# ZhangHaoyang493/News_Recsys

Measured on AMD Instinct MI355X. Metric: impressions/sec at batch 65536 (embedding hot path forward), higher is better.
Workload: dtype f32

## Files before the change

news_recsys_amd/csrc/nrx_interact.hip:

```cpp
#include "nrx_common.h"

namespace {

__global__ __launch_bounds__(NRX_BLOCK) void bag_pool_fwd_kernel(const float* __restrict__ emb, const float* __restrict__ mask,
                                                                 int64_t batch, int L, int D, float* __restrict__ out) {
    const int64_t total = batch * (int64_t)D;
    for (int64_t i = (int64_t)blockIdx.x * NRX_BLOCK + threadIdx.x; i < total; i += (int64_t)gridDim.x * NRX_BLOCK) {
        const int64_t b = i / D;
        const int d = (int)(i - b * D);
        const float* e = emb + (b * L) * (int64_t)D + d;
        float acc = 0.f, den = 0.f;
        if (mask != nullptr) {
            const float* m = mask + b * (int64_t)L;
            for (int l = 0; l < L; ++l) {
#pragma clang fp contract(off)
                const float w = m[l];
                den += w;
                acc += e[(int64_t)l * D] * w;
            }
            out[i] = acc / (den + 1e-8f);
        } else {
            for (int l = 0; l < L; ++l) acc += e[(int64_t)l * D];
            out[i] = acc / (float)L;
        }
    }
}

template <bool VEC>
__global__ __launch_bounds__(NRX_BLOCK) void bag_pool_bwd_kernel(const float* __restrict__ g_out, const float* __restrict__ mask,
                                                                 int64_t batch, int L, int D, float* __restrict__ g_emb) {
    const int lane = threadIdx.x & 63;
    const int64_t wave = (int64_t)blockIdx.x * (NRX_BLOCK / 64) + (threadIdx.x >> 6);
    const int64_t nwaves = (int64_t)gridDim.x * (NRX_BLOCK / 64);
    const int n = L * D;
    for (int64_t b = wave; b < batch; b += nwaves) {
        float den = (float)L;
        if (mask != nullptr) {
            float part = 0.f;
            for (int l = lane; l < L; l += NRX_WAVE) part += mask[b * (int64_t)L + l];
            den = nrx_wave_sum(part) + 1e-8f;
        }
        const float* gb = g_out + b * (int64_t)D;
        const float* mb = mask ? mask + b * (int64_t)L : nullptr;
        float* ob = g_emb + b * (int64_t)n;
        if (VEC) {
            const unsigned q = (unsigned)D >> 2;
            for (unsigned e4 = lane; e4 < (unsigned)n >> 2; e4 += NRX_WAVE) {
                const unsigned l = e4 / q, d = (e4 - l * q) * 4;
                const float4 g = *reinterpret_cast<const float4*>(gb + d);
                const float m = mb ? mb[l] : 1.0f;
                float4 o = make_float4(g.x / den, g.y / den, g.z / den, g.w / den);
                if (mb) o = make_float4(o.x * m, o.y * m, o.z * m, o.w * m);
                *reinterpret_cast<float4*>(ob + (size_t)e4 * 4) = o;
            }
        } else {
            for (int e = lane; e < n; e += NRX_WAVE) {
                const int l = e / D, d = e - l * D;
                const float g = gb[d] / den;
                ob[e] = mb ? g * mb[l] : g;
            }
        }
    }
}

__device__ __forceinline__ float4 ld4(const float* p, int k0, int D, bool vec) {
    float4 v;
    if (vec) {
        v = *reinterpret_cast<const float4*>(p);
    } else {
        v.x = p[0];
        v.y = (k0 + 1 < D) ? p[1] : 0.f;
        v.z = (k0 + 2 < D) ? p[2] : 0.f;
        v.w = (k0 + 3 < D) ? p[3] : 0.f;
    }
    return v;
}

template <int QLOG2>
__global__ __launch_bounds__(NRX_BLOCK) void fm_fwd_kernel(const float* __restrict__ feat, int64_t ld, int F, int D,
                                                           int64_t batch, float* __restrict__ fm_out, bool vec,
                                                           float* __restrict__ sums = nullptr, int64_t sums_ld = 0) {
    constexpr int Q = 1 << QLOG2;
    constexpr int TB = NRX_BLOCK / Q;
    const int q = threadIdx.x & (Q - 1);
    const int64_t b = (int64_t)blockIdx.x * TB + (threadIdx.x >> QLOG2);
    const bool live = b < batch;
    float total = 0.f;
    for (int kc = 0; kc < D; kc += 4 * Q) {
        const int k0 = kc + q * 4;
        float first = 0.f;
        float4 s = make_float4(0.f, 0.f, 0.f, 0.f), sq = s;
        if (live && k0 < D) {
            const float* row = feat + b * ld + k0;
            for (int f = 0; f < F; ++f) {
                float4 v = ld4(row + (int64_t)f * D, k0, D, vec);
                if (k0 == 0) { first += v.x; v.x = 0.f; }
                s.x += v.x; s.y += v.y; s.z += v.z; s.w += v.w;
                sq.x += v.x * v.x; sq.y += v.y * v.y; sq.z += v.z * v.z; sq.w += v.w * v.w;
            }
        }
        total += 0.5f * ((s.x * s.x - sq.x) + (s.y * s.y - sq.y) + (s.z * s.z - sq.z) + (s.w * s.w - sq.w)) + first;
        if (sums != nullptr && live && k0 < D) {
            float* dst = sums + b * sums_ld + k0;
            const float v0 = k0 == 0 ? first : s.x;
            dst[0] = v0;
            if (k0 + 1 < D) dst[1] = s.y;
            if (k0 + 2 < D) dst[2] = s.z;
            if (k0 + 3 < D) dst[3] = s.w;
        }
    }
#pragma unroll
    for (int off = Q / 2; off > 0; off >>= 1) total += __shfl_xor(total, off, 64);
    if (live && q == 0) fm_out[b] = total;
}

template <int QLOG2>
__global__ __launch_bounds__(NRX_BLOCK) void fm_bwd_kernel(const float* __restrict__ feat, int64_t ld, int F, int D, int64_t batch,
                                                           const float* __restrict__ g_fm, const float* g_in, int64_t g_in_ld,
                                                           float* g_feat, int64_t g_ld, bool vec) {
    constexpr int Q = 1 << QLOG2;
    constexpr int TB = NRX_BLOCK / Q;
    constexpr int U = 8;
    const int q = threadIdx.x & (Q - 1);
    const int64_t b = (int64_t)blockIdx.x * TB + (threadIdx.x >> QLOG2);
    if (b >= batch) return;
    const float gl = g_fm[b];
    const bool gvec = vec && (g_ld & 3) == 0 && ((reinterpret_cast<uintptr_t>(g_feat) & 15u) == 0) &&
                      (g_in == nullptr || ((g_in_ld & 3) == 0 && (reinterpret_cast<uintptr_t>(g_in) & 15u) == 0));
    for (int kc = 0; kc < D; kc += 4 * Q) {
        const int k0 = kc + q * 4;
        if (k0 >= D) continue;
        const float* row = feat + b * ld + k0;
        const float* irow = g_in ? g_in + b * g_in_ld + k0 : nullptr;
        float* grow = g_feat + b * g_ld + k0;
        float4 s = make_float4(0.f, 0.f, 0.f, 0.f);
        int f = 0;
        for (; f + U <= F; f += U) {
            float4 v[U];
#pragma unroll
            for (int u = 0; u < U; ++u) v[u] = ld4(row + (int64_t)(f + u) * D, k0, D, vec);
#pragma unroll
            for (int u = 0; u < U; ++u) { s.x += v[u].x; s.y += v[u].y; s.z += v[u].z; s.w += v[u].w; }
        }
        for (; f < F; ++f) {
            const float4 v = ld4(row + (int64_t)f * D, k0, D, vec);
            s.x += v.x; s.y += v.y; s.z += v.z; s.w += v.w;
        }
        f = 0;
        if (gvec && k0 + 4 <= D) {
            for (; f + U <= F; f += U) {
                float4 v[U], up[U];
#pragma unroll
                for (int u = 0; u < U; ++u) {
                    v[u] = ld4(row + (int64_t)(f + u) * D, k0, D, vec);
                    up[u] = irow ? *reinterpret_cast<const float4*>(irow + (int64_t)(f + u) * D) : make_float4(0.f, 0.f, 0.f, 0.f);
                }
#pragma unroll
                for (int u = 0; u < U; ++u) {
                    float4 g = make_float4(gl * (s.x - v[u].x), gl * (s.y - v[u].y), gl * (s.z - v[u].z), gl * (s.w - v[u].w));
                    if (k0 == 0) g.x = gl;
                    *reinterpret_cast<float4*>(grow + (int64_t)(f + u) * D) = make_float4(up[u].x + g.x, up[u].y + g.y, up[u].z + g.z, up[u].w + g.w);
                }
            }
        }
        for (; f < F; ++f) {
            const float4 v = ld4(row + (int64_t)f * D, k0, D, vec);
            float g[4] = {gl * (s.x - v.x), gl * (s.y - v.y), gl * (s.z - v.z), gl * (s.w - v.w)};
            if (k0 == 0) g[0] = gl;
            float* gp = grow + (int64_t)f * D;
            const float* ip = irow ? irow + (int64_t)f * D : nullptr;
#pragma unroll
            for (int j = 0; j < 4; ++j)
                if (k0 + j < D) gp[j] = (ip ? ip[j] : 0.f) + g[j];
        }
    }
}

template <int R, int V>
struct RowRegs {
    float v[R][V];
};

template <int R, int V>
__device__ __forceinline__ void row_load(RowRegs<R, V>& x, const float* p, int D, int lane) {
#pragma unroll
    for (int r = 0; r < R; ++r) {
        const int c = (r * 64 + lane) * V;
        if (V == 4) {
            float4 t = make_float4(0.f, 0.f, 0.f, 0.f);
            if (c < D) t = *reinterpret_cast<const float4*>(p + c);
            x.v[r][0] = t.x; x.v[r][1 % V] = t.y; x.v[r][2 % V] = t.z; x.v[r][3 % V] = t.w;
        } else {
            x.v[r][0] = (c < D) ? p[c] : 0.f;
        }
    }
}
// ... 499 lines not shown
                if (STNT) __builtin_nontemporal_store(t, o + u * Q + q);
                else o[u * Q + q] = t;
            }
        }
        float4 xl[N];
#pragma unroll
        for (int u = 0; u < N; ++u) xl[u] = x0[u];
        for (int l = 0; l < NL; ++l) {
            const float4* wl = s_w + l * (W / 4) + q;
            const float4* bl = s_b + l * (W / 4) + q;
            float part = 0.f;
#pragma unroll
            for (int u = 0; u < N; ++u) {
                const float4 wv = wl[u * Q];
                part += xl[u].x * wv.x + xl[u].y * wv.y + xl[u].z * wv.z + xl[u].w * wv.w;
            }
            const float dot = group_sum_dpp<Q>(part);
#pragma unroll
            for (int u = 0; u < N; ++u) {
                const float4 bv = bl[u * Q];
                xl[u].x = x0[u].x * dot + bv.x + xl[u].x;
                xl[u].y = x0[u].y * dot + bv.y + xl[u].y;
                xl[u].z = x0[u].z * dot + bv.z + xl[u].z;
                xl[u].w = x0[u].w * dot + bv.w + xl[u].w;
            }
        }
        if (live) {
            NRX_GLOBAL nrx_f32x4* o = (NRX_GLOBAL nrx_f32x4*)(a->out + b * a->out_ld);
#pragma unroll
            for (int u = EARLY ? N : 0; u < 2 * N; ++u) {
                const float4 v = u < N ? x0[u] : xl[u - N];
                nrx_f32x4 t;
                t.x = v.x; t.y = v.y; t.z = v.z; t.w = v.w;
                NRX_GLOBAL nrx_f32x4* dst = o + (u < N ? 0 : W / 4) + (u < N ? u : u - N) * Q + q;
                if (STNT) __builtin_nontemporal_store(t, dst);
                else *dst = t;
            }
        }
    }
}

int ceil_log2i(int x) {
    int l = 0;
    while ((1 << l) < x) ++l;
    return l;
}

unsigned stream_grid(int64_t items, int per_block) {
    int64_t g = (items + per_block - 1) / per_block;
    const int64_t cap = 256 * 8;
    if (g > cap) g = cap;
    if (g < 1) g = 1;
    return (unsigned)g;
}

#define NRX_QSWITCH(qlog2, ...)               \
    switch (qlog2) {                           \
        case 0: { constexpr int QL = 0; __VA_ARGS__; } break; \
        case 1: { constexpr int QL = 1; __VA_ARGS__; } break; \
        case 2: { constexpr int QL = 2; __VA_ARGS__; } break; \
        case 3: { constexpr int QL = 3; __VA_ARGS__; } break; \
        case 4: { constexpr int QL = 4; __VA_ARGS__; } break; \
        case 5: { constexpr int QL = 5; __VA_ARGS__; } break; \
        default: { constexpr int QL = 6; __VA_ARGS__; } break; \
    }

#define NRX_RSWITCH(R_, V_, ...)                                   \
    if (V_ == 4) {                                                  \
        constexpr int VV = 4;                                       \
        if (R_ <= 1) { constexpr int RR = 1; __VA_ARGS__; }                \
        else if (R_ <= 2) { constexpr int RR = 2; __VA_ARGS__; }           \
        else if (R_ <= 4) { constexpr int RR = 4; __VA_ARGS__; }           \
        else { constexpr int RR = 8; __VA_ARGS__; }                        \
    } else {                                                        \
        constexpr int VV = 1;                                       \
        if (R_ <= 1) { constexpr int RR = 1; __VA_ARGS__; }                \
        else if (R_ <= 2) { constexpr int RR = 2; __VA_ARGS__; }           \
        else if (R_ <= 4) { constexpr int RR = 4; __VA_ARGS__; }           \
        else if (R_ <= 8) { constexpr int RR = 8; __VA_ARGS__; }           \
        else if (R_ <= 16) { constexpr int RR = 16; __VA_ARGS__; }         \
        else { constexpr int RR = 32; __VA_ARGS__; }                       \
    }

}

extern "C" int nrx_bag_pool_fwd(const float* emb, const float* mask, int64_t batch, int32_t bag_len,
                                int32_t dim, float* out, void* stream) {
    NRX_TRACE();
    NRX_REQUIRE(emb && out && batch >= 0 && bag_len >= 1 && dim >= 1, "nrx_bag_pool_fwd: bad argument");
    if (batch == 0) return NRX_OK;
    hipLaunchKernelGGL(bag_pool_fwd_kernel, dim3(stream_grid(batch * dim, NRX_BLOCK)), dim3(NRX_BLOCK), 0,
                       reinterpret_cast<hipStream_t>(stream), emb, mask, batch, bag_len, dim, out);
    NRX_LAUNCH_CHECK("nrx_bag_pool_fwd");
    return NRX_OK;
}

extern "C" int nrx_bag_pool_bwd(const float* g_out, const float* mask, int64_t batch, int32_t bag_len,
                                int32_t dim, float* g_emb, void* stream) {
    NRX_TRACE();
    NRX_REQUIRE(g_out && g_emb && batch >= 0 && bag_len >= 1 && dim >= 1, "nrx_bag_pool_bwd: bad argument");
    if (batch == 0) return NRX_OK;
    const bool vec = (dim & 3) == 0 && nrx_aligned16(g_out) && nrx_aligned16(g_emb);
    if (vec) hipLaunchKernelGGL(bag_pool_bwd_kernel<true>, dim3(stream_grid(batch, NRX_BLOCK / 64)), dim3(NRX_BLOCK), 0,
                                reinterpret_cast<hipStream_t>(stream), g_out, mask, batch, bag_len, dim, g_emb);
    else hipLaunchKernelGGL(bag_pool_bwd_kernel<false>, dim3(stream_grid(batch, NRX_BLOCK / 64)), dim3(NRX_BLOCK), 0,
                            reinterpret_cast<hipStream_t>(stream), g_out, mask, batch, bag_len, dim, g_emb);
    NRX_LAUNCH_CHECK("nrx_bag_pool_bwd");
    return NRX_OK;
}

extern "C" int nrx_fm_fwd(const float* feat, int64_t ld, int32_t n_fields, int32_t dim, int64_t batch,
                          float* fm_out, void* stream) {
    NRX_TRACE();
    NRX_REQUIRE(feat && fm_out && n_fields >= 1 && dim >= 1 && batch >= 0 && ld >= (int64_t)n_fields * dim,
                "nrx_fm_fwd: bad argument");
    if (batch == 0) return NRX_OK;
    int ql = ceil_log2i((dim + 3) / 4);
    if (ql > 6) ql = 6;
    const bool vec = (dim & 3) == 0 && (ld & 3) == 0 && nrx_aligned16(feat);
    const int tb = NRX_BLOCK >> ql;
    const unsigned grid = (unsigned)((batch + tb - 1) / tb);
    NRX_QSWITCH(ql, { hipLaunchKernelGGL((fm_fwd_kernel<QL>), dim3(grid), dim3(NRX_BLOCK), 0, reinterpret_cast<hipStream_t>(stream),
                                         feat, ld, n_fields, dim, batch, fm_out, vec); });
    NRX_LAUNCH_CHECK("nrx_fm_fwd");
    return NRX_OK;
}

extern "C" int nrx_fm_fwd_train(const float* feat, int64_t ld, int32_t n_fields, int32_t dim, int64_t batch,
                                float* fm_out, float* fm_sums, int64_t sums_ld, void* stream) {
    NRX_TRACE();
    NRX_REQUIRE(feat && fm_out && fm_sums && n_fields >= 1 && dim >= 1 && batch >= 0 && ld >= (int64_t)n_fields * dim && sums_ld >= dim,
                "nrx_fm_fwd_train: bad argument");
    if (batch == 0) return NRX_OK;
    int ql = ceil_log2i((dim + 3) / 4);
    if (ql > 6) ql = 6;
    const bool vec = (dim & 3) == 0 && (ld & 3) == 0 && nrx_aligned16(feat);
    const int tb = NRX_BLOCK >> ql;
    const unsigned grid = (unsigned)((batch + tb - 1) / tb);
    NRX_QSWITCH(ql, { hipLaunchKernelGGL((fm_fwd_kernel<QL>), dim3(grid), dim3(NRX_BLOCK), 0, reinterpret_cast<hipStream_t>(stream),
                                         feat, ld, n_fields, dim, batch, fm_out, vec, fm_sums, sums_ld); });
    NRX_LAUNCH_CHECK("nrx_fm_fwd_train");
    return NRX_OK;
}

extern "C" int nrx_fm_bwd(const float* feat, int64_t ld, int32_t n_fields, int32_t dim, int64_t batch,
                          const float* g_fm, const float* g_in, int64_t g_in_ld, float* g_feat, int64_t g_ld, void* stream) {
    NRX_TRACE();
    NRX_REQUIRE(feat && g_fm && g_feat && n_fields >= 1 && dim >= 1 && batch >= 0, "nrx_fm_bwd: bad argument");
    if (batch == 0) return NRX_OK;
    int ql = ceil_log2i((dim + 3) / 4);
    if (ql > 6) ql = 6;
    const bool vec = (dim & 3) == 0 && (ld & 3) == 0 && nrx_aligned16(feat);
    const int tb = NRX_BLOCK >> ql;
    const unsigned grid = (unsigned)((batch + tb - 1) / tb);
    NRX_QSWITCH(ql, { hipLaunchKernelGGL((fm_bwd_kernel<QL>), dim3(grid), dim3(NRX_BLOCK), 0, reinterpret_cast<hipStream_t>(stream),
                                         feat, ld, n_fields, dim, batch, g_fm, g_in, g_in_ld, g_feat, g_ld, vec); });
    NRX_LAUNCH_CHECK("nrx_fm_bwd");
    return NRX_OK;
}

namespace {
constexpr int FH_BLOCKS = 64;
__global__ __launch_bounds__(NRX_BLOCK) void fm_head_fwd_kernel(const float* __restrict__ logit, const float* __restrict__ bias, float* __restrict__ out,
                                                                int64_t batch) {
    const float b = bias != nullptr ? bias[0] : 0.f;
    for (int64_t i = (int64_t)blockIdx.x * NRX_BLOCK + threadIdx.x; i < batch; i += (int64_t)gridDim.x * NRX_BLOCK) {
        const float x = b + logit[i];
        out[i] = 1.0f / (1.0f + expf(-x));
    }
}
__global__ __launch_bounds__(NRX_BLOCK) void fm_head_bwd_kernel(const float* __restrict__ g_out, int64_t g_stride, const float* __restrict__ out,
                                                                float* __restrict__ g_logit, float* __restrict__ g_bias, uint32_t* __restrict__ state,
                                                                int64_t batch) {
    __shared__ float s_w[NRX_BLOCK / 64];
    __shared__ uint32_t s_last;
    const int64_t chunk = (batch + gridDim.x - 1) / gridDim.x;
    const int64_t lo = (int64_t)blockIdx.x * chunk, hi = lo + chunk < batch ? lo + chunk : batch;
    float acc = 0.f;
    for (int64_t i = lo + threadIdx.x; i < hi; i += NRX_BLOCK) {
        const float p = out[i];
        const float g = g_out[i * g_stride] * (p * (1.0f - p));
        g_logit[i] = g;
        acc += g;
    }
    if (g_bias == nullptr) return;
    acc = nrx_wave_sum(acc);
    if ((threadIdx.x & 63) == 0) s_w[threadIdx.x >> 6] = acc;
    __syncthreads();
    float* partial = reinterpret_cast<float*>(state + 8);
    if (threadIdx.x == 0) {
        partial[blockIdx.x] = (s_w[0] + s_w[1]) + (s_w[2] + s_w[3]);
        __threadfence();
        s_last = atomicAdd(&state[0], 1u) == gridDim.x - 1 ? 1u : 0u;
    }
    __syncthreads();
    if (s_last && threadIdx.x < 64) {
        __threadfence();
        float v = (int)threadIdx.x < (int)gridDim.x ? __hip_atomic_load(&partial[threadIdx.x], __ATOMIC_RELAXED, __HIP_MEMORY_SCOPE_AGENT) : 0.f;
        v = nrx_wave_sum(v);
        if (threadIdx.x == 0) {
            g_bias[0] = v;
            state[0] = 0;
        }
    }
}
}

extern "C" int nrx_fm_head_fwd(const float* logit, const float* bias, float* out, int64_t batch, void* stream) {
    NRX_TRACE();
    NRX_REQUIRE(logit && out && batch >= 0, "nrx_fm_head_fwd: bad argument");
    if (batch == 0) return NRX_OK;
    const int64_t g = (batch + NRX_BLOCK - 1) / NRX_BLOCK;
    hipLaunchKernelGGL(fm_head_fwd_kernel, dim3((unsigned)(g < 1024 ? g : 1024)), dim3(NRX_BLOCK), 0, reinterpret_cast<hipStream_t>(stream), logit, bias, out, batch);
    NRX_LAUNCH_CHECK("nrx_fm_head_fwd");
    return NRX_OK;
}

extern "C" int64_t nrx_fm_head_state_bytes(void) { return 32 + FH_BLOCKS * 4; }

extern "C" int nrx_fm_head_bwd(const float* g_out, int64_t g_stride, const float* out, float* g_logit, float* g_bias, void* state, int64_t batch,
                               void* stream) {
    NRX_TRACE();
    NRX_REQUIRE(g_out && out && g_logit && batch >= 0 && (g_stride == 0 || g_stride == 1), "nrx_fm_head_bwd: bad argument");
// ... 322 lines not shown
```

news_recsys_amd/csrc/nrx_route_feat.hip:

```cpp
#include <cstring>

#include "nrx_common.h"

namespace {

constexpr int RF_THREADS = 256;
#ifndef NRX_RF_ROUNDS
#define NRX_RF_ROUNDS 16
#endif
constexpr int RF_ROUNDS = NRX_RF_ROUNDS;
constexpr int RF_TILE = RF_THREADS * RF_ROUNDS;
constexpr int RF_WAVES = RF_THREADS / 64;
constexpr int RF_MAX_WORLD = 64;

struct RouteFeatArgs {
    const void* ids[NRX_MAX_FEATURES];
    int64_t batch;
    int64_t capf;
    int32_t n_feats, world, idx64, tiles;
    int32_t* send_ids;
    int32_t* send_pos;
    int32_t* slot;
    int64_t* counts;
    int64_t* overflow;
    uint32_t* ctl;
    unsigned long long* agg;
    int32_t use_ticket;
};
static_assert(sizeof(RouteFeatArgs) <= 3584, "kernarg budget");

__global__ __launch_bounds__(RF_THREADS) void route_feat_kernel(const RouteFeatArgs args_in_kernarg) {
    const NRX_CONST RouteFeatArgs* a = nrx_kernarg<RouteFeatArgs>();
    __shared__ int s_cell[RF_ROUNDS * RF_WAVES][RF_MAX_WORLD];
    __shared__ int s_tot[RF_MAX_WORLD], s_base[RF_MAX_WORLD];
    __shared__ uint32_t s_ticket, s_mark;
    const int tid = threadIdx.x, lane = tid & 63, wid = tid >> 6;
    const int W = a->world, n = a->n_feats, T = a->tiles;
    if (W == 1) {
        const int f = (int)blockIdx.x / T, tile = (int)blockIdx.x - f * T;
        const int64_t B = a->batch, i0 = (int64_t)tile * RF_TILE, capf = a->capf;
        const void* p = a->ids[f];
#pragma unroll
        for (int j = 0; j < RF_ROUNDS; ++j) {
            const int64_t i = i0 + j * RF_THREADS + tid;
            if (i >= B) continue;
            const int64_t id = a->idx64 ? nrx_gconst<int64_t>(p)[i] : (int64_t)nrx_gconst<int32_t>(p)[i];
            const int32_t v = id < 0 ? -1 : id >= 0x7fffffffLL ? 0x7fffffff : id == 0 ? 0 : (int32_t)(id + 1);
            if (i < capf) {
                a->send_ids[(int64_t)f * capf + i] = v;
                if (a->send_pos != nullptr) a->send_pos[(int64_t)f * capf + i] = (int32_t)i;
                a->slot[(int64_t)f * B + i] = (int32_t)(i * n + f);
            } else {
                a->slot[(int64_t)f * B + i] = -1;
            }
        }
        if (tile == T - 1) {
            if (tid == 0) {
                a->counts[f] = B;
                atomicMax(reinterpret_cast<long long*>(a->overflow), (long long)B);
            }
            for (int64_t k = B + tid; k < capf; k += RF_THREADS) {
                a->send_ids[(int64_t)f * capf + k] = 0;
                if (a->send_pos != nullptr) a->send_pos[(int64_t)f * capf + k] = -1;
            }
        }
        return;
    }
    if (tid == 0) {
        s_ticket = a->use_ticket ? atomicAdd(&a->ctl[0], 1u) : blockIdx.x;
        s_mark = __hip_atomic_load(&a->ctl[2], __ATOMIC_RELAXED, __HIP_MEMORY_SCOPE_AGENT) + 1u;
    }
    if (tid < RF_MAX_WORLD) s_base[tid] = 0;
    __syncthreads();
    const int w = (int)s_ticket;
    const uint32_t mark = s_mark;
    const int f = w / T, tile = w - f * T;
    const int64_t B = a->batch, i0 = (int64_t)tile * RF_TILE;
    int owner[RF_ROUNDS];
    int32_t val[RF_ROUNDS];
    {
        const void* p = a->ids[f];
        int64_t id[RF_ROUNDS];
#pragma unroll
        for (int j = 0; j < RF_ROUNDS; ++j) {
            const int64_t i = i0 + j * RF_THREADS + tid;
// ... 387 lines not shown
struct GatherPlaceArgs {
    const float* table[NRX_MAX_FEATURES];
    int64_t rows[NRX_MAX_FEATURES];
    int32_t col[NRX_MAX_FEATURES];
    float* peer[RF_MAX_WORLD];
    const int32_t* oid;
    const int32_t* opos;
    int64_t bp, capf, ld, out_rows;
    int32_t n, world;
    int32_t* status;
};
static_assert(sizeof(GatherPlaceArgs) <= 3584, "kernarg budget");

typedef unsigned nrx_gp_u32x2 __attribute__((ext_vector_type(2)));
template <int QLOG2, typename TS = float>
__global__ __launch_bounds__(NRX_BLOCK) void gather_place_feat_kernel(const GatherPlaceArgs args_in_kernarg) {
    const NRX_CONST GatherPlaceArgs* a = nrx_kernarg<GatherPlaceArgs>();
    constexpr int Q = 1 << QLOG2, TB = NRX_BLOCK / Q;
    const int q = threadIdx.x & (Q - 1);
    const int64_t bp = a->bp;
    const int n = a->n;
    for (int64_t b = (int64_t)blockIdx.x * TB + (threadIdx.x >> QLOG2); b < bp; b += (int64_t)gridDim.x * TB) {
        const int s = (int)(b / a->capf);
        float* __restrict__ out = a->peer[s];
        auto fetch = [&](int f0, int32_t* id, int32_t* pos) {
#pragma unroll
            for (int r = 0; r < GP_R; ++r) {
                const int f = f0 + r < n ? f0 + r : n - 1;
                id[r] = nrx_gconst<int32_t>(a->oid)[(int64_t)f * bp + b];
                pos[r] = nrx_gconst<int32_t>(a->opos)[(int64_t)f * bp + b];
            }
        };
        auto process = [&](int f0, const int32_t* id, int32_t* pos) {
            float4 v[GP_R];
            [[maybe_unused]] nrx_gp_u32x2 raw[GP_R];
            [[maybe_unused]] bool use[GP_R];
#pragma unroll
            for (int r = 0; r < GP_R; ++r) {
                const int f = f0 + r < n ? f0 + r : n - 1;
                v[r] = make_float4(0.f, 0.f, 0.f, 0.f);
                if constexpr (sizeof(TS) == 2) {
                    const uint64_t tb = reinterpret_cast<uint64_t>(a->table[f]);
                    const uint32_t tb_lo = __builtin_amdgcn_readfirstlane((uint32_t)tb), tb_hi = __builtin_amdgcn_readfirstlane((uint32_t)(tb >> 32));
                    const uint32_t nr = __builtin_amdgcn_readfirstlane((uint32_t)(a->rows[f] > 0x7fffffff ? 0x7fffffff : a->rows[f]));
                    const NRX_GLOBAL nrx_gp_u32x2* base = (const NRX_GLOBAL nrx_gp_u32x2*)(((uint64_t)tb_hi << 32) | tb_lo);
                    use[r] = f0 + r < n && pos[r] >= 0 && id[r] > 0 && (uint32_t)id[r] < nr;
                    raw[r] = __builtin_nontemporal_load(base + ((int64_t)(use[r] ? id[r] : 0) * Q + q));
                }
                if (f0 + r >= n || pos[r] < 0) { pos[r] = -1; continue; }
                if (id[r] < 0 || (int64_t)id[r] >= a->rows[f]) {
                    if (q == 0) nrx_report_oob(a->status, f, b, id[r]);
                    continue;
                }
                if constexpr (sizeof(TS) != 2) {
                    if (id[r] != 0) v[r] = nrx_ldg4_nt(a->table[f], (int64_t)id[r] * Q + q);
                }
            }
#pragma unroll
            for (int r = 0; r < GP_R; ++r) {
                if (pos[r] < 0) continue;
                const int f = f0 + r;
                if ((int64_t)pos[r] >= a->out_rows) {
                    if (q == 0) nrx_report_oob(a->status, f, b, pos[r]);
                    continue;
                }
                if constexpr (sizeof(TS) == 2) {
                    if (use[r]) v[r] = nrx_bf16x4_to_f32(raw[r].x, raw[r].y);
                }
                nrx_stg4(out, ((int64_t)pos[r] * a->ld + a->col[f]) / 4 + q, v[r]);
            }
        };
        int32_t ida[GP_R], posa[GP_R], idb[GP_R], posb[GP_R];
        fetch(0, ida, posa);
        for (int f0 = 0; f0 < n; f0 += 2 * GP_R) {
            if (f0 + GP_R < n) fetch(f0 + GP_R, idb, posb);
            process(f0, ida, posa);
            if (f0 + GP_R >= n) break;
            if (f0 + 2 * GP_R < n) fetch(f0 + 2 * GP_R, ida, posa);
            process(f0 + GP_R, idb, posb);
        }
    }
}

__global__ __launch_bounds__(NRX_BLOCK) void shard_dest_combine_kernel(const int32_t* __restrict__ slot, const int32_t* __restrict__ dest_req, int n, int64_t batch,
                                                                      int64_t capf, int64_t recv_row0, int rank, int shift, int32_t* __restrict__ out) {
    const int f = blockIdx.y;
    const uint32_t un = (uint32_t)n, ucapf = (uint32_t)capf;
    for (int64_t b = (int64_t)blockIdx.x * NRX_BLOCK + threadIdx.x; b < batch; b += (int64_t)gridDim.x * NRX_BLOCK) {
        const int64_t p = (int64_t)f * batch + b;
        const int32_t sl = slot[p];
        int32_t r = -1;
        if (sl >= 0) {
            const uint32_t ok = (uint32_t)sl / un, o = ok / ucapf, k = ok - o * ucapf;
            const int32_t d = dest_req[((int64_t)o * n + f) * capf + k];
            const int64_t row = d >= 0 ? (int64_t)d : recv_row0 + ((int64_t)rank * capf + k) * n + f;
            r = (int32_t)(((int64_t)o << shift) | row);
        }
        out[p] = r;
    }
}

bool all_resident(const void* kernel, int64_t blocks) {
    static thread_local const void* cached_k[4] = {nullptr, nullptr, nullptr, nullptr};
    static thread_local int64_t cached_cap[4] = {0, 0, 0, 0};
    int64_t capacity = -1;
    for (int i = 0; i < 4; ++i)
        if (cached_k[i] == kernel) capacity = cached_cap[i];
    if (capacity < 0) {
        int per_cu = 0, dev = 0, cus = 0;
        if (hipOccupancyMaxActiveBlocksPerMultiprocessor(&per_cu, kernel, RF_THREADS, 0) != hipSuccess || hipGetDevice(&dev) != hipSuccess ||
            hipDeviceGetAttribute(&cus, hipDeviceAttributeMultiprocessorCount, dev) != hipSuccess)
            return false;
        capacity = (int64_t)per_cu * cus;
        for (int i = 0; i < 4; ++i)
            if (cached_k[i] == nullptr) { cached_k[i] = kernel; cached_cap[i] = capacity; break; }
    }
    return blocks <= capacity;
}

}

extern "C" int nrx_shard_dest_combine(const int32_t* slot, const int32_t* dest_req, int32_t n_feats, int64_t batch, int64_t capf, int64_t recv_row0,
                                      int32_t rank, int32_t world, int32_t shift, int32_t* dest_out, void* stream) {
    NRX_TRACE();
    NRX_REQUIRE(slot && dest_req && dest_out && n_feats >= 1 && batch >= 0 && capf >= 1 && rank >= 0 && rank < world, "nrx_shard_dest_combine: bad argument");
    NRX_REQUIRE(shift >= 1 && shift <= 30 && (int64_t)world <= (1ll << (31 - shift)) && recv_row0 + (int64_t)world * capf * n_feats <= (1ll << shift),
                "nrx_shard_dest_combine: (owner << shift) | row must fit 31 bits");
    if (batch == 0) return NRX_OK;
    NRX_REQUIRE(capf < 0x7fffffffLL && n_feats <= NRX_MAX_FEATURES, "nrx_shard_dest_combine: capf must fit 31 bits, n_feats <= %d", NRX_MAX_FEATURES);
    int64_t blocks = (batch + NRX_BLOCK - 1) / NRX_BLOCK;
    if (blocks > 1024) blocks = 1024;
    hipLaunchKernelGGL(shard_dest_combine_kernel, dim3((unsigned)blocks, (unsigned)n_feats), dim3(NRX_BLOCK), 0, reinterpret_cast<hipStream_t>(stream), slot, dest_req, (int)n_feats,
                       batch, capf, recv_row0, (int)rank, (int)shift, dest_out);
    NRX_LAUNCH_CHECK("nrx_shard_dest_combine");
    return NRX_OK;
}

namespace {
template <typename TS>
int gather_place_feat_launch(const char* who, const void* const* tables, const int64_t* table_rows, const int32_t* feat_col, int32_t n_feats, int32_t world,
                                     int64_t capf, const int32_t* owner_ids, const int32_t* owner_pos, int32_t dim, float* const* peer_out,
                                     int64_t out_ld, int64_t out_rows, int32_t* status, void* stream) {
    NRX_REQUIRE(tables && table_rows && feat_col && owner_ids && owner_pos && peer_out, "%s: null argument", who);
    NRX_REQUIRE(n_feats >= 1 && n_feats <= NRX_MAX_FEATURES && world >= 1 && world <= RF_MAX_WORLD && capf >= 1, "%s: bad sizes", who);
    if (!(dim == 16 || dim == 32 || dim == 64 || dim == 128 || dim == 256) || (out_ld & 3) != 0) {
        nrx_set_error("%s: dim must be 16 / 32 / 64 / 128 / 256 and out_ld a multiple of 4", who);
        return NRX_ERR_UNSUPPORTED;
    }
    GatherPlaceArgs a;
    memset(&a, 0, sizeof(a));
    for (int i = 0; i < n_feats; ++i) {
        NRX_REQUIRE(tables[i] != nullptr && (reinterpret_cast<uintptr_t>(tables[i]) & (sizeof(TS) == 2 ? 7u : 15u)) == 0 && (feat_col[i] & 3) == 0,
                    "%s: feature %d: aligned table and column", who, i);
        NRX_REQUIRE(sizeof(TS) != 2 || table_rows[i] >= 1, "%s: feature %d: a bf16 arena has at least its dummy row", who, i);
        a.table[i] = reinterpret_cast<const float*>(tables[i]);
        a.rows[i] = table_rows[i];
        a.col[i] = feat_col[i];
    }
    for (int s = 0; s < world; ++s) {
        NRX_REQUIRE(peer_out[s] != nullptr && nrx_aligned16(peer_out[s]), "%s: peer %d: null / unaligned buffer", who, s);
        a.peer[s] = peer_out[s];
    }
    a.oid = owner_ids;
    a.opos = owner_pos;
    a.bp = (int64_t)world * capf;
    a.capf = capf;
    a.ld = out_ld;
    a.out_rows = out_rows;
    a.n = n_feats;
    a.world = world;
    a.status = status;
    const int ql = dim == 16 ? 2 : dim == 32 ? 3 : dim == 64 ? 4 : dim == 128 ? 5 : 6;
    const int64_t tb = NRX_BLOCK >> ql;
    int64_t blocks = (a.bp + tb - 1) / tb;
    if (blocks > 8192) blocks = 8192;
    hipStream_t st = reinterpret_cast<hipStream_t>(stream);
    if (ql == 2) hipLaunchKernelGGL((gather_place_feat_kernel<2, TS>), dim3((unsigned)blocks), dim3(NRX_BLOCK), 0, st, a);
    else if (ql == 3) hipLaunchKernelGGL((gather_place_feat_kernel<3, TS>), dim3((unsigned)blocks), dim3(NRX_BLOCK), 0, st, a);
    else if (ql == 4) hipLaunchKernelGGL((gather_place_feat_kernel<4, TS>), dim3((unsigned)blocks), dim3(NRX_BLOCK), 0, st, a);
    else if (ql == 5) hipLaunchKernelGGL((gather_place_feat_kernel<5, TS>), dim3((unsigned)blocks), dim3(NRX_BLOCK), 0, st, a);
    else hipLaunchKernelGGL((gather_place_feat_kernel<6, TS>), dim3((unsigned)blocks), dim3(NRX_BLOCK), 0, st, a);
    NRX_LAUNCH_CHECK(who);
    return NRX_OK;
}
}

extern "C" int nrx_gather_place_feat(const float* const* tables, const int64_t* table_rows, const int32_t* feat_col, int32_t n_feats, int32_t world,
                                     int64_t capf, const int32_t* owner_ids, const int32_t* owner_pos, int32_t dim, float* const* peer_out,
                                     int64_t out_ld, int64_t out_rows, int32_t* status, void* stream) {
    NRX_TRACE();
    return gather_place_feat_launch<float>("nrx_gather_place_feat", reinterpret_cast<const void* const*>(tables), table_rows, feat_col, n_feats, world, capf,
                                           owner_ids, owner_pos, dim, peer_out, out_ld, out_rows, status, stream);
}

extern "C" int nrx_gather_place_feat_bf16(const uint16_t* const* tables, const int64_t* table_rows, const int32_t* feat_col, int32_t n_feats, int32_t world,
                                          int64_t capf, const int32_t* owner_ids, const int32_t* owner_pos, int32_t dim, float* const* peer_out,
                                          int64_t out_ld, int64_t out_rows, int32_t* status, void* stream) {
    NRX_TRACE();
    return gather_place_feat_launch<uint16_t>("nrx_gather_place_feat_bf16", reinterpret_cast<const void* const*>(tables), table_rows, feat_col, n_feats, world,
                                              capf, owner_ids, owner_pos, dim, peer_out, out_ld, out_rows, status, stream);
}

extern "C" int64_t nrx_route_feat_state_bytes(int32_t n_feats, int64_t batch, int32_t world) {
    if (n_feats < 1 || n_feats > NRX_MAX_FEATURES || batch < 0 || world < 1 || world > RF_MAX_WORLD) return -1;
    const int64_t tiles = (batch + RF_TILE - 1) / RF_TILE;
    return 512 + (int64_t)n_feats * (tiles > 0 ? tiles : 1) * world * 8;
}

extern "C" int nrx_route_feat(const void* const* ids, int32_t n_feats, int64_t batch, int32_t index_bits, int32_t world, int64_t capf,
                              int32_t* send_ids, int32_t* send_pos, int32_t* slot, int64_t* counts, int64_t* overflow, void* state, void* stream) {
    NRX_TRACE();
    NRX_REQUIRE(ids != nullptr && n_feats >= 1 && n_feats <= NRX_MAX_FEATURES, "nrx_route_feat: n_feats must be in [1, %d]", NRX_MAX_FEATURES);
    NRX_REQUIRE(world >= 1 && world <= RF_MAX_WORLD, "nrx_route_feat: world must be in [1, %d]", RF_MAX_WORLD);
    NRX_REQUIRE(index_bits == 32 || index_bits == 64, "nrx_route_feat: index_bits must be 32 or 64");
    NRX_REQUIRE(batch >= 0 && batch < 0x7fffffffLL && capf >= 1, "nrx_route_feat: bad batch / capf");
    NRX_REQUIRE((int64_t)world * capf * n_feats < 0x7fffffffLL, "nrx_route_feat: world * capf * n_feats must stay below 2^31 (slot is int32)");
    NRX_REQUIRE(send_ids && slot && counts && overflow && state, "nrx_route_feat: null buffer");
    if (batch == 0) return NRX_OK;
    RouteFeatArgs a;
    memset(&a, 0, sizeof(a));
    for (int i = 0; i < n_feats; ++i) {
        NRX_REQUIRE(ids[i] != nullptr, "nrx_route_feat: feature %d: null ids", i);
        a.ids[i] = ids[i];
    }
    a.batch = batch;
    a.capf = capf;
    a.n_feats = n_feats;
    a.world = world;
    a.idx64 = index_bits == 64;
    a.tiles = (int32_t)((batch + RF_TILE - 1) / RF_TILE);
    a.send_ids = send_ids;
    a.send_pos = send_pos;
    a.slot = slot;
    a.counts = counts;
    a.overflow = overflow;
    a.ctl = reinterpret_cast<uint32_t*>(state);
    a.agg = reinterpret_cast<unsigned long long*>(reinterpret_cast<char*>(state) + 512);
    a.use_ticket = world > 1 && !all_resident(reinterpret_cast<const void*>(route_feat_kernel), (int64_t)n_feats * a.tiles);
    hipLaunchKernelGGL(route_feat_kernel, dim3((unsigned)(n_feats * a.tiles)), dim3(RF_THREADS), 0, reinterpret_cast<hipStream_t>(stream), a);
    NRX_LAUNCH_CHECK("nrx_route_feat");
    return NRX_OK;
}

extern "C" int64_t nrx_route_bags_one_state_bytes(const int32_t* bag_lens, int32_t n_feats, int64_t batch, int32_t world) {
    if (bag_lens == nullptr || n_feats < 1 || n_feats > NRX_MAX_FEATURES || batch < 0 || world < 1 || world > RF_MAX_WORLD) return -1;
    int64_t tiles = 0;
    for (int f = 0; f < n_feats; ++f) tiles += (batch * bag_lens[f] + RF_TILE - 1) / RF_TILE;
    return 64 + ((tiles > 0 ? tiles : 1) + tiles / RB_GROUP + 1) * world * 8;
}

extern "C" int nrx_route_bags_one(const void* const* ids, const float* const* weights, const int32_t* bag_lens, int32_t n_feats, int32_t index_bits,
                                  int64_t batch, int32_t world, int64_t cap, int32_t* send_rows, int32_t* send_tag, float* send_w, int64_t* counts2d,
                                  int64_t* overflow, void* state, void* stream) {
    NRX_TRACE();
    NRX_REQUIRE(ids && bag_lens && n_feats >= 1 && n_feats <= NRX_MAX_FEATURES, "nrx_route_bags_one: n_feats must be in [1, %d]", NRX_MAX_FEATURES);
    NRX_REQUIRE(index_bits == 32 || index_bits == 64, "nrx_route_bags_one: index_bits must be 32 or 64");
    NRX_REQUIRE(world >= 1 && world <= RF_MAX_WORLD && cap >= 1 && cap * world <= 0x7fffffffLL && batch >= 0, "nrx_route_bags_one: bad world / cap / batch");
    NRX_REQUIRE((int64_t)n_feats * batch <= 0x7fffffffLL, "nrx_route_bags_one: n_feats * batch must fit 31 bits");
    NRX_REQUIRE(send_rows && send_tag && send_w && counts2d && overflow && state, "nrx_route_bags_one: null buffer");
// ... 122 lines not shown
```

Before: 1.098 billion.

## Add in-flight FM forward kernels and LDS-staged ring gather-place kernel

```diff
diff --git a/news_recsys_amd/csrc/nrx_interact.hip b/news_recsys_amd/csrc/nrx_interact.hip
--- a/news_recsys_amd/csrc/nrx_interact.hip
+++ b/news_recsys_amd/csrc/nrx_interact.hip
@@ -74,6 +74,30 @@
         v.w = (k0 + 3 < D) ? p[3] : 0.f;
     }
     return v;
+}
+
+__device__ __forceinline__ void fm_pass_add(float4 v, int k0, float& first, float4& s, float4& sq) {
+    if (k0 == 0) { first += v.x; v.x = 0.f; }
+    s.x += v.x; s.y += v.y; s.z += v.z; s.w += v.w;
+    sq.x = __builtin_fmaf(v.x, v.x, sq.x); sq.y = __builtin_fmaf(v.y, v.y, sq.y);
+    sq.z = __builtin_fmaf(v.z, v.z, sq.z); sq.w = __builtin_fmaf(v.w, v.w, sq.w);
+}
+__device__ __forceinline__ void fm_pass_part(float& total, const float4& s, const float4& sq, float first) {
+    const float a = __builtin_fmaf(s.x, s.x, -sq.x), b = __builtin_fmaf(s.y, s.y, -sq.y);
+    float c, d;
+    {
+#pragma clang fp contract(off)
+        c = s.z * s.z - sq.z;
+        d = s.w * s.w - sq.w;
+    }
+    total += __builtin_fmaf(0.5f, ((a + b) + c) + d, first);
+}
+__device__ __forceinline__ void fm_pass_write_sums(float* dst, int k0, int D, const float4& s, float first) {
+    const float v0 = k0 == 0 ? first : s.x;
+    dst[0] = v0;
+    if (k0 + 1 < D) dst[1] = s.y;
+    if (k0 + 2 < D) dst[2] = s.z;
+    if (k0 + 3 < D) dst[3] = s.w;
 }
 
 template <int QLOG2>
@@ -112,6 +136,81 @@
 #pragma unroll
     for (int off = Q / 2; off > 0; off >>= 1) total += __shfl_xor(total, off, 64);
     if (live && q == 0) fm_out[b] = total;
+}
+
+constexpr int FM_U = 8;
+template <int QLOG2>
+__global__ __launch_bounds__(NRX_BLOCK) void fm_fwd_inflight_kernel(const float* __restrict__ feat, int64_t ld, int F, int D,
+                                                                    int64_t batch, float* __restrict__ fm_out, bool vec,
+                                                                    float* __restrict__ sums, int64_t sums_ld) {
+    constexpr int Q = 1 << QLOG2;
+    constexpr int TB = NRX_BLOCK / Q;
+    const int q = threadIdx.x & (Q - 1);
+    const int64_t b = (int64_t)blockIdx.x * TB + (threadIdx.x >> QLOG2);
+    const bool live = b < batch;
+    float total = 0.f;
+    for (int kc = 0; kc < D; kc += 4 * Q) {
+        const int k0 = kc + q * 4;
+        float first = 0.f;
+        float4 s = make_float4(0.f, 0.f, 0.f, 0.f), sq = s;
+        if (live && k0 < D) {
+            const float* row = feat + b * ld + k0;
+            if (vec) {
+                for (int f0 = 0; f0 < F; f0 += FM_U) {
+                    float4 v[FM_U];
+#pragma unroll
+                    for (int u = 0; u < FM_U; ++u) {
+                        const int f = f0 + u < F ? f0 + u : F - 1;
+                        v[u] = *reinterpret_cast<const float4*>(row + (int64_t)f * D);
+                    }
+                    __builtin_amdgcn_sched_barrier(0);
+#pragma unroll
+                    for (int u = 0; u < FM_U; ++u)
+                        if (f0 + u < F) fm_pass_add(v[u], k0, first, s, sq);
+                }
+            } else {
+                for (int f = 0; f < F; ++f) fm_pass_add(ld4(row + (int64_t)f * D, k0, D, false), k0, first, s, sq);
+            }
+        }
+        fm_pass_part(total, s, sq, first);
+        if (sums != nullptr && live && k0 < D) fm_pass_write_sums(sums + b * sums_ld + k0, k0, D, s, first);
+    }
+#pragma unroll
+    for (int off = Q / 2; off > 0; off >>= 1) total += __shfl_xor(total, off, 64);
+    if (live && q == 0) fm_out[b] = total;
+}
+
+template <int NJ>
+__global__ __launch_bounds__(NRX_BLOCK) void fm_fwd_lines_kernel(const float* __restrict__ feat, int64_t ld, int F, int64_t batch,
+                                                                 float* __restrict__ fm_out, float* __restrict__ sums, int64_t sums_ld) {
+    constexpr int D = 16, TB = NRX_BLOCK / 8;
+    const int q = threadIdx.x & 3, h = (threadIdx.x >> 2) & 1;
+    const int64_t b = (int64_t)blockIdx.x * TB + (threadIdx.x >> 3);
+    if (b >= batch) return;
+    const int k0 = q * 4;
+    const float* row = feat + b * ld + k0;
+    float total = 0.f, first = 0.f;
+    float4 s = make_float4(0.f, 0.f, 0.f, 0.f), sq = s;
+    for (int f0 = 0; f0 < F; f0 += 2 * NJ) {
+        float4 v[NJ];
+#pragma unroll
+        for (int j = 0; j < NJ; ++j) {
+            const int f = f0 + 2 * j + h < F ? f0 + 2 * j + h : F - 1;
+            v[j] = *reinterpret_cast<const float4*>(row + (int64_t)f * D);
+        }
+        __builtin_amdgcn_sched_barrier(0);
+#pragma unroll
+        for (int j = 0; j < NJ; ++j) {
+            const float4 w = make_float4(nrx_dpp<0x104>(v[j].x), nrx_dpp<0x104>(v[j].y), nrx_dpp<0x104>(v[j].z), nrx_dpp<0x104>(v[j].w));
+            if (f0 + 2 * j < F) fm_pass_add(v[j], k0, first, s, sq);
+            if (f0 + 2 * j + 1 < F) fm_pass_add(w, k0, first, s, sq);
+        }
+    }
+    fm_pass_part(total, s, sq, first);
+    if (sums != nullptr && h == 0) fm_pass_write_sums(sums + b * sums_ld + k0, k0, D, s, first);
+    total += __shfl_xor(total, 2, 64);
+    total += __shfl_xor(total, 1, 64);
+    if (h == 0 && q == 0) fm_out[b] = total;
 }
 
 template <int QLOG2>
@@ -777,6 +876,34 @@
         else { constexpr int RR = 32; __VA_ARGS__; }                       \
     }
 
+void fm_fwd_launch(const float* feat, int64_t ld, int32_t n_fields, int32_t dim, int64_t batch, float* fm_out, float* fm_sums, int64_t sums_ld,
+                   hipStream_t st) {
+    int ql = ceil_log2i((dim + 3) / 4);
+    if (ql > 6) ql = 6;
+    const bool vec = (dim & 3) == 0 && (ld & 3) == 0 && nrx_aligned16(feat);
+    const int tb = NRX_BLOCK >> ql;
+    const unsigned grid = (unsigned)((batch + tb - 1) / tb);
+    const char* e = getenv("NRX_FM_FWD_FORM");
+    if ((e != nullptr && atoi(e) == 0) || ql == 0) {
+        NRX_QSWITCH(ql, { hipLaunchKernelGGL((fm_fwd_kernel<QL>), dim3(grid), dim3(NRX_BLOCK), 0, st, feat, ld, n_fields, dim, batch, fm_out, vec, fm_sums, sums_ld); });
+        return;
+    }
+    if (dim == 16 && (ld & 31) == 0 && (reinterpret_cast<uintptr_t>(feat) & 127u) == 0) {
+        const unsigned lgrid = (unsigned)((batch + NRX_BLOCK / 8 - 1) / (NRX_BLOCK / 8));
+        const int need = (n_fields + 1) / 2;
+#define NRX_FM_LINES(NJ_) hipLaunchKernelGGL((fm_fwd_lines_kernel<NJ_>), dim3(lgrid), dim3(NRX_BLOCK), 0, st, feat, ld, n_fields, batch, fm_out, fm_sums, sums_ld)
+        if (need <= 1) NRX_FM_LINES(1);
+        else if (need <= 2) NRX_FM_LINES(2);
+        else if (need <= 4) NRX_FM_LINES(4);
+        else if (need <= 8) NRX_FM_LINES(8);
+        else if (need <= 13) NRX_FM_LINES(13);
+        else NRX_FM_LINES(16);
+#undef NRX_FM_LINES
+        return;
+    }
+    NRX_QSWITCH(ql, { hipLaunchKernelGGL((fm_fwd_inflight_kernel<QL>), dim3(grid), dim3(NRX_BLOCK), 0, st, feat, ld, n_fields, dim, batch, fm_out, vec, fm_sums, sums_ld); });
+}
+
 }
 
 extern "C" int nrx_bag_pool_fwd(const float* emb, const float* mask, int64_t batch, int32_t bag_len,
@@ -810,13 +937,7 @@
     NRX_REQUIRE(feat && fm_out && n_fields >= 1 && dim >= 1 && batch >= 0 && ld >= (int64_t)n_fields * dim,
                 "nrx_fm_fwd: bad argument");
     if (batch == 0) return NRX_OK;
-    int ql = ceil_log2i((dim + 3) / 4);
-    if (ql > 6) ql = 6;
-    const bool vec = (dim & 3) == 0 && (ld & 3) == 0 && nrx_aligned16(feat);
-    const int tb = NRX_BLOCK >> ql;
-    const unsigned grid = (unsigned)((batch + tb - 1) / tb);
-    NRX_QSWITCH(ql, { hipLaunchKernelGGL((fm_fwd_kernel<QL>), dim3(grid), dim3(NRX_BLOCK), 0, reinterpret_cast<hipStream_t>(stream),
-                                         feat, ld, n_fields, dim, batch, fm_out, vec); });
+    fm_fwd_launch(feat, ld, n_fields, dim, batch, fm_out, nullptr, 0, reinterpret_cast<hipStream_t>(stream));
     NRX_LAUNCH_CHECK("nrx_fm_fwd");
     return NRX_OK;
 }
@@ -827,13 +948,7 @@
     NRX_REQUIRE(feat && fm_out && fm_sums && n_fields >= 1 && dim >= 1 && batch >= 0 && ld >= (int64_t)n_fields * dim && sums_ld >= dim,
                 "nrx_fm_fwd_train: bad argument");
     if (batch == 0) return NRX_OK;
-    int ql = ceil_log2i((dim + 3) / 4);
-    if (ql > 6) ql = 6;
-    const bool vec = (dim & 3) == 0 && (ld & 3) == 0 && nrx_aligned16(feat);
-    const int tb = NRX_BLOCK >> ql;
-    const unsigned grid = (unsigned)((batch + tb - 1) / tb);
-    NRX_QSWITCH(ql, { hipLaunchKernelGGL((fm_fwd_kernel<QL>), dim3(grid), dim3(NRX_BLOCK), 0, reinterpret_cast<hipStream_t>(stream),
-                                         feat, ld, n_fields, dim, batch, fm_out, vec, fm_sums, sums_ld); });
+    fm_fwd_launch(feat, ld, n_fields, dim, batch, fm_out, fm_sums, sums_ld, reinterpret_cast<hipStream_t>(stream));
     NRX_LAUNCH_CHECK("nrx_fm_fwd_train");
     return NRX_OK;
 }
diff --git a/news_recsys_amd/csrc/nrx_route_feat.hip b/news_recsys_amd/csrc/nrx_route_feat.hip
--- a/news_recsys_amd/csrc/nrx_route_feat.hip
+++ b/news_recsys_amd/csrc/nrx_route_feat.hip
@@ -1,6 +1,7 @@
 #include <cstring>
 
 #include "nrx_common.h"
+#include "nrx_embed_ring.h"
 
 namespace {
 
@@ -554,6 +555,119 @@
     }
 }
 
+template <int QLOG2, int R, bool NT, typename TS, bool PRED>
+__device__ __forceinline__ void gather_place_walk(const NRX_CONST GatherPlaceArgs* a, const int2* s_my, int n, int q, float* out, int64_t ld4) {
+    using nrx_ring::load_row;
+    constexpr int TB = NRX_BLOCK >> QLOG2;
+    auto uni = [](int f) { return __builtin_amdgcn_readfirstlane(f); };
+    auto place = [&](int f, int2 rec, float4 v) {
+        if (PRED && rec.y < 0) return;
+        if (rec.x == 0) v = make_float4(0.f, 0.f, 0.f, 0.f);
+        nrx_stg4(out, (int64_t)rec.y * ld4 + (a->col[uni(f)] >> 2) + q, v);
+    };
+    float4 v[R];
+    int2 rec[R];
+#pragma unroll
+    for (int u = 0; u < R; ++u) rec[u] = s_my[u * TB];
+#pragma unroll
+    for (int u = 0; u < R; ++u) v[u] = load_row<QLOG2, NT, TS>(a->table[u], rec[u].x, q);
+    int f0 = 0;
+    for (; f0 + 2 * R <= n; f0 += R) {
+        int2 nxt[R];
+#pragma unroll
+        for (int u = 0; u < R; ++u) nxt[u] = s_my[(f0 + R + u) * TB];
+#pragma unroll
+        for (int u = 0; u < R; ++u) {
+            place(f0 + u, rec[u], v[u]);
+            rec[u] = nxt[u];
+            v[u] = load_row<QLOG2, NT, TS>(a->table[uni(f0 + R + u)], nxt[u].x, q);
+            __builtin_amdgcn_sched_barrier(0);
+        }
+    }
+    {
+        int2 nxt[R];
+#pragma unroll
+        for (int u = 0; u < R; ++u) {
+            const int f = f0 + R + u;
+            nxt[u] = s_my[(f < n ? f : n - 1) * TB];
+        }
+#pragma unroll
+        for (int u = 0; u < R; ++u) {
+            place(f0 + u, rec[u], v[u]);
+            if (f0 + R + u < n) {
+                rec[u] = nxt[u];
+                v[u] = load_row<QLOG2, NT, TS>(a->table[uni(f0 + R + u)], nxt[u].x, q);
+            }
+            __builtin_amdgcn_sched_barrier(0);
+        }
+#pragma unroll
+        for (int u = 0; u < R; ++u)
+            if (f0 + R + u < n) place(f0 + R + u, rec[u], v[u]);
+    }
+}
+
+template <int QLOG2, int R, bool NT, typename TS>
+__global__ __launch_bounds__(NRX_BLOCK, 4) void gather_place_ring_kernel(const GatherPlaceArgs args_in_kernarg) {
+    const NRX_CONST GatherPlaceArgs* a = nrx_kernarg<GatherPlaceArgs>();
+    constexpr int Q = 1 << QLOG2, TB = NRX_BLOCK / Q;
+    extern __shared__ __attribute__((aligned(16))) int2 s_rec[];
+    __shared__ int s_holes;
+    const int tid = threadIdx.x, n = a->n;
+    const int64_t bp = a->bp, b0 = (int64_t)blockIdx.x * TB;
+    const int nb = (int)(bp - b0 < (int64_t)TB ? bp - b0 : (int64_t)TB);
+    if (tid == 0) s_holes = 0;
+    __syncthreads();
+    {
+        const int lane = tid & (NRX_WAVE - 1);
+        const int wave = __builtin_amdgcn_readfirstlane(tid >> 6);
+        const int sl = lane < nb ? lane : nb - 1;
+        const int64_t out_rows = a->out_rows;
+        constexpr int PASS = 4;
+        bool holes = false;
+        for (int k0 = 0; k0 * 4 < n; k0 += PASS) {
+            int32_t idv[PASS], posv[PASS];
+#pragma unroll
+            for (int u = 0; u < PASS; ++u) {
+                int f = (k0 + u) * 4 + wave;
+                f = f < n ? f : n - 1;
+                idv[u] = nrx_gconst<int32_t>(a->oid)[(int64_t)f * bp + b0 + sl];
+                posv[u] = nrx_gconst<int32_t>(a->opos)[(int64_t)f * bp + b0 + sl];
+            }
+#pragma unroll
+            for (int u = 0; u < PASS; ++u) {
+                const int f = (k0 + u) * 4 + wave;
+                const int fc = f < n ? f : n - 1;
+                const bool mine = f < n && lane < nb;
+                int32_t row = 0, pos = -1;
+                if (mine && posv[u] >= 0) {
+                    row = idv[u];
+                    pos = posv[u];
+                    if (row < 0 || (int64_t)row >= a->rows[fc]) {
+                        nrx_report_oob(a->status, f, b0 + lane, row);
+                        row = 0;
+                    }
+                    if ((int64_t)pos >= out_rows) {
+                        nrx_report_oob(a->status, f, b0 + lane, pos);
+                        pos = -1;
+                    }
+                }
+                if (mine && pos < 0) holes = true;
+                if (f < n && lane < TB) s_rec[f * TB + lane] = make_int2(row, pos);
+            }
+        }
+        if (holes) s_holes = 1;
+    }
+    __syncthreads();
+    const int q = tid & (Q - 1), sb = tid >> QLOG2;
+    const int64_t b = b0 + sb;
+    if (b >= bp) return;
+    float* out = a->peer[(int)(b / a->capf)];
+    const int2* s_my = s_rec + sb;
+    const int64_t ld4 = a->ld >> 2;
+    if (__builtin_amdgcn_readfirstlane(s_holes) != 0) gather_place_walk<QLOG2, R, NT, TS, true>(a, s_my, n, q, out, ld4);
+    else gather_place_walk<QLOG2, R, NT, TS, false>(a, s_my, n, q, out, ld4);
+}
+
 __global__ __launch_bounds__(NRX_BLOCK) void shard_dest_combine_kernel(const int32_t* __restrict__ slot, const int32_t* __restrict__ dest_req, int n, int64_t batch,
                                                                       int64_t capf, int64_t recv_row0, int rank, int shift, int32_t* __restrict__ out) {
     const int f = blockIdx.y;
@@ -645,8 +759,42 @@
     const int ql = dim == 16 ? 2 : dim == 32 ? 3 : dim == 64 ? 4 : dim == 128 ? 5 : 6;
     const int64_t tb = NRX_BLOCK >> ql;
     int64_t blocks = (a.bp + tb - 1) / tb;
+    hipStream_t st = reinterpret_cast<hipStream_t>(stream);
+    bool ring = blocks <= 0x7fffffffLL;
+    { const char* e = getenv("NRX_GATHER_PLACE_FORM"); if (e != nullptr && atoi(e) == 0) ring = false; }
+    int64_t arena_bytes = 0;
+    for (int i = 0; i < n_feats; ++i) {
+        if (table_rows[i] < 1) ring = false;
+        arena_bytes += table_rows[i] * (int64_t)dim * (int64_t)sizeof(TS);
+    }
+    if (ring) {
+        bool nt = arena_bytes > (256ll << 20);
+        { const char* e = getenv("NRX_GATHER_PLACE_NT"); if (e != nullptr) nt = atoi(e) != 0; }
+        const int r = (n_feats >= 8 && !(ql == 2 && nt)) ? 8 : n_feats >= 4 ? 4 : 1;
+        const dim3 grid((unsigned)blocks), block(NRX_BLOCK);
+        const size_t lds = (size_t)n_feats * tb * sizeof(int2);
+#define NRX_GPR(QL_, R_)                                                                                                 \
+    do {                                                                                                                 \
+        if (nt) hipLaunchKernelGGL((gather_place_ring_kernel<QL_, R_, true, TS>), grid, block, lds, st, a);              \
+        else hipLaunchKernelGGL((gather_place_ring_kernel<QL_, R_, false, TS>), grid, block, lds, st, a);                \
+    } while (0)
+#define NRX_GPQ(QL_)                                                                                                     \
+    do {                                                                                                                 \
+        if (r == 8) NRX_GPR(QL_, 8);                                                                                     \
+        else if (r == 4) NRX_GPR(QL_, 4);                                                                                \
+        else NRX_GPR(QL_, 1);                                                                                            \
+    } while (0)
+        if (ql == 2) NRX_GPQ(2);
+        else if (ql == 3) NRX_GPQ(3);
+        else if (ql == 4) NRX_GPQ(4);
+        else if (ql == 5) NRX_GPQ(5);
+        else NRX_GPQ(6);
+#undef NRX_GPQ
+#undef NRX_GPR
+        NRX_LAUNCH_CHECK(who);
+        return NRX_OK;
+    }
     if (blocks > 8192) blocks = 8192;
-    hipStream_t st = reinterpret_cast<hipStream_t>(stream);
     if (ql == 2) hipLaunchKernelGGL((gather_place_feat_kernel<2, TS>), dim3((unsigned)blocks), dim3(NRX_BLOCK), 0, st, a);
     else if (ql == 3) hipLaunchKernelGGL((gather_place_feat_kernel<3, TS>), dim3((unsigned)blocks), dim3(NRX_BLOCK), 0, st, a);
     else if (ql == 4) hipLaunchKernelGGL((gather_place_feat_kernel<4, TS>), dim3((unsigned)blocks), dim3(NRX_BLOCK), 0, st, a);
```

Result: no change. 1.097 billion (-0.1%).
